# huggingface/tokenizers

Measured on AMD Instinct MI355X. Metric: GB input text/sec (whole node), GPT-2 BPE encode_batch, higher is better.
Workload: dtype u8->u32

## Files before the change

### tokenizers_amd/csrc/capi/handle.cpp

```cpp

struct Workspace {
    std::mutex mu;
    std::function<uint32_t(uint32_t)> pad_exchange;
    uint32_t h_padmax = 0;
    bool busy = false;
    bool device_bound = false;
    hipStream_t bound_stream = nullptr;
    hipStream_t own_stream = nullptr;
    hipStream_t io_in = nullptr, io_out = nullptr;
    hipEvent_t ev_in[2] = {nullptr, nullptr}, ev_out[2] = {nullptr, nullptr};
    DevBuf w_l3_tiles;
    DevBuf w_ms_dmask, w_pprefix, w_pt_word;
    DevBuf w_docmask, w_startmask, w_wprefix, w_bsum, w_tile_w, w_pt_start, w_tok0, w_pt_tokoff, w_tmp_ids, w_tmp_end, w_rows;
    DevBuf w_len1, w_fin, w_fbsum, w_pad_count, w_keep, w_type_ids2, w_seq_ids2;
    DevBuf w_ovf_parts, w_enc_base, w_enc_doc, w_enc_start, w_enc_cnt;
    DevBuf w_enc_idx, w_enc_win;
    DevBuf w_queues, w_qcount, w_cstate;
    DevBuf w_doc_off;
    DevBuf w_chunk_lo;
    DevBuf w_ids, w_doc_pt, w_tok_offsets, w_scalars, w_offsets, w_word_ids;
    DevBuf dw_ids, dw_tok_off, dw_first, dw_bad, dw_dup, dw_len, dw_bsum, dw_pos, dw_out_off, dw_bytes, dw_total;
    DevBuf w_endmask, w_pt_end, w_keepmask, w_kprefix, w_ntext, w_norig, w_ndoc_off, w_slow_docs, w_leadmask, w_lprefix, w_need, w_need_bsum, w_huge, w_list_huge, w_wbase, w_norig_e, w_ids2, w_tok_offsets2, w_offsets2, w_word_ids2, w_candmask, w_matchmask, w_spanmask, w_stopmask, w_hardmask, w_boundmask, w_bprefix, w_seg_off, w_xseg_off,
        w_match_docs, w_match_list;
    DevBuf h_text, h_doc_off, h_seq_off, h_inp_off;
    DevBuf w_tok_b8;
    DevBuf w_trim1;
    const uint8_t* cur_trim1 = nullptr;
    DevBuf w_cache_keys, w_cache_rows;
    DevBuf w_claims, w_claim_rows, w_claim_pos;
    DevBuf w_phases;
    uint64_t cache_epoch = 0;
    DevBuf w_seq_off, w_seq_tok_off, w_word_idx, w_first_tok;
    std::vector<StageRec> pending;
    const uint8_t* last_text = nullptr;
    const int64_t* last_doc_off = nullptr;
    const int64_t* last_seq_off = nullptr;
    int64_t last_n_seqs = -1;
    const int64_t* last_inp_off = nullptr;
    int64_t last_n_inputs = -1;
    DevBuf w_inp_off;
    DevBuf w_mask_dirty;
    int64_t last_n_bytes = 0;
    uint32_t last_flags = 0;
    tkamd_device_result last_result{};
    int64_t last_n_docs = 0;
    int64_t last_n_enc = -1;
    int last_ntok_slot = 1;
    uint32_t last_counters[CNT_COUNT] = {0};
    bool force_general = false;
    bool force_nfc = false;
    bool last_note_nfc = false;
    bool last_note_added = false;
    bool last_used_claims = false;
    ~Workspace() {
        if (own_stream) (void)hipStreamDestroy(own_stream);
        if (io_in) (void)hipStreamDestroy(io_in);
        if (io_out) (void)hipStreamDestroy(io_out);
        for (int i = 0; i < 2; ++i) {
            if (ev_in[i]) (void)hipEventDestroy(ev_in[i]);
            if (ev_out[i]) (void)hipEventDestroy(ev_out[i]);
        }
    }
};

struct tkamd_tokenizer {
    HostModel hm;
    int device = -1;
    DevTables dt{};
    std::mutex mu;
    std::condition_variable cv;
    std::vector<std::unique_ptr<Workspace>> pool;
    Workspace* last_used = nullptr;
    DevBuf t_ucc1, t_ucc2;
    DevBuf t_uc1, t_uc2, t_byte_id, t_merges, t_long_blob, t_long_off, t_long_id, t_long_table;
    DevBuf t_hot;
    DevBuf t_shortw, t_shortw_k3, t_shortw_disp;
    DevBuf t_char_id;
    DevBuf t_at_id[2], t_at_flags[2], t_at_blob[2], t_at_off[2], t_at_first[2];
    DevBuf t_pp_single, t_pp_single_plain;
    DevBuf t_pp_pair, t_pp_pair_plain;
    DevBuf t_pp_prefix, t_pp_suffix, t_pp_prefix_ty, t_pp_suffix_ty, t_bn1, t_bn2, t_bn_map, t_nfc1, t_nfc2, t_nfc_map, t_merge_disp, t_dec_entry, t_dec_blob, t_trie;
    int n_cu = 256;
    int n_direct = 0;
    int n_hot = 0;
    int cp_grid = 0;
    std::atomic<int> claims_pause{0};
    std::atomic<int> added_spec_pause{0};
    std::atomic<int> nfc_spec_pause{0};
    std::atomic<uint32_t> nfc_reruns{0};
    int nfc_spec_len = 32;
    int added_spec_len = 32;
    int claims_pause_len = 32;
    std::atomic<uint32_t> q16_div{4};
    std::atomic<bool> prof{false};
    std::atomic<bool> encode_special{false};
    std::atomic<bool> word_cache{false};
    std::atomic<uint64_t> cache_epoch{1};
    std::vector<tkamd_stage_time> acc;
    std::vector<int> devices;
    std::vector<std::unique_ptr<tkamd_tokenizer>> replicas;
    std::mutex group_mu;
    std::atomic<int> collect{0};
    std::string collect_note;
    std::vector<std::unique_ptr<DevBuf>> g_root;
    std::vector<void*> rccl_comms;
    int64_t shard_min_bytes = 1 << 20;
    std::vector<double> shard_ms;
    std::vector<int64_t> shard_bytes;
};

constexpr size_t PHASE_WGS = 1 << 17;
constexpr size_t MAX_HOST_WORKSPACES = 4;

struct PinnedBlock {
    void* p = nullptr;
    size_t cap = 0;
};
static std::mutex g_pin_mu;
static std::vector<PinnedBlock> g_pin_free;

static PinnedBlock pinned_get(size_t bytes) {
    if (bytes < 64) bytes = 64;
    {
        std::lock_guard<std::mutex> lk(g_pin_mu);
        size_t best = (size_t)-1;
        for (size_t i = 0; i < g_pin_free.size(); ++i)
            if (g_pin_free[i].cap >= bytes && (best == (size_t)-1 || g_pin_free[i].cap < g_pin_free[best].cap)) best = i;
        if (best != (size_t)-1 && g_pin_free[best].cap <= 2 * bytes + (1u << 20)) {
            PinnedBlock b = g_pin_free[best];
            g_pin_free.erase(g_pin_free.begin() + best);
            return b;
        }
    }
    PinnedBlock b;
    size_t want = bytes + bytes / 8;
    HIP_CHECK(hipHostMalloc(&b.p, want, hipHostMallocPortable));
    b.cap = want;
    return b;
}
static void pinned_put(PinnedBlock b) {
    if (!b.p || g_forked) return;
    std::lock_guard<std::mutex> lk(g_pin_mu);
    if (g_pin_free.size() >= 16) { (void)hipHostFree(b.p); return; }
    g_pin_free.push_back(b);
}

struct tkamd_batch {
    int64_t n_docs = 0, n_tokens = 0;
    PinnedBlock ids, tok_offsets, offsets, word_ids, pad_counts, type_ids, seq_ids, enc_docs, enc_parts;
    bool has_offsets = false, has_words = false, has_pads = false, has_types = false, has_enc_docs = false, has_enc_parts = false;
    ~tkamd_batch() { pinned_put(ids); pinned_put(tok_offsets); pinned_put(offsets); pinned_put(word_ids); pinned_put(pad_counts); pinned_put(type_ids); pinned_put(seq_ids); pinned_put(enc_docs); pinned_put(enc_parts); }
};

struct tkamd_text {
    int64_t n_docs = 0, n_bytes = 0;
    PinnedBlock bytes, doc_offsets;
    ~tkamd_text() { pinned_put(bytes); pinned_put(doc_offsets); }
};
```

### tokenizers_amd/csrc/capi/probes.cpp

```cpp

int tkamd_probe_word(const tkamd_tokenizer* t, const uint8_t* bytes, int32_t len, uint32_t* id, uint32_t* flags) {
    if (!t || !bytes || !id || !flags || len < 0) return set_error(TKAMD_ERR_INVALID, "bad argument");
    const HostModel& hm = t->hm;
    *id = 0;
    *flags = 0;
    if (len == 0 || hm.word_table.empty()) return 0;
    if (len <= WORD_MAX_KEY) {
        uint8_t buf[16] = {0};
        memcpy(buf, bytes, (size_t)len);
        uint64_t lo, hi;
        memcpy(&lo, buf, 8);
        memcpy(&hi, buf + 8, 8);
        const uint32_t h1 = word_hash1(lo, hi, (uint32_t)len, hm.word_seed);
        const WordSlot& sa = hm.word_table[word_slot_a(h1, hm.word_mask)];
        const WordSlot& s = (sa.len == (uint32_t)len && sa.lo == lo && sa.hi == hi) ? sa : hm.word_table[word_slot_b(h1, hm.word_mask)];
        if (s.len != (uint32_t)len || s.lo != lo || s.hi != hi) return 0;
        *id = s.id;
        *flags = s.flags;
        return 1;
    }
    if (hm.long_table.empty()) return 0;
    uint32_t h = fnv1a(bytes, (size_t)len) & hm.long_mask;
    for (;;) {
        const uint32_t e = hm.long_table[h];
// ... 92 lines not shown
    t->encode_special = value != 0;
    for (auto& r : t->replicas) r->encode_special = value != 0;
    return TKAMD_OK;
}

int tkamd_word_cache(tkamd_tokenizer* t, int enable, int clear) {
    if (!t) return set_error(TKAMD_ERR_INVALID, "null argument");
    if (clear) ++t->cache_epoch;
    t->word_cache = enable != 0;
    for (auto& r : t->replicas) { if (clear) ++r->cache_epoch; r->word_cache = enable != 0; }
    return TKAMD_OK;
}

int tkamd_profile_enable(tkamd_tokenizer* t, int on) {
    if (!t) return set_error(TKAMD_ERR_INVALID, "null argument");
    t->prof = on != 0;
    for (auto& r : t->replicas) r->prof = on != 0;
    return TKAMD_OK;
}

int tkamd_profile_read(tkamd_tokenizer* t, tkamd_stage_time* stages, int max_stages, int* n_stages, int reset) {
    if (!t || !n_stages) return set_error(TKAMD_ERR_INVALID, "null argument");
    std::lock_guard<std::mutex> lk(t->mu);
    if (t->device >= 0 && !g_forked) {
        (void)hipSetDevice(t->device);
        for (auto& w : t->pool) drain_profile(t, w.get());
        for (auto& r : t->replicas) {
            std::lock_guard<std::mutex> rl(r->mu);
            (void)hipSetDevice(r->device);
            for (auto& w : r->pool) drain_profile(t, w.get());
        }
        if (!t->replicas.empty()) (void)hipSetDevice(t->device);
    }
    int n = (int)std::min<size_t>(t->acc.size(), (size_t)std::max(0, max_stages));
    for (int i = 0; i < n && stages; ++i) stages[i] = t->acc[i];
    *n_stages = n;
    if (reset) t->acc.clear();
    return TKAMD_OK;
}

int tkamd_pinned_alloc(size_t bytes, void** out) {
    if (!out) return set_error(TKAMD_ERR_INVALID, "null argument");
    *out = nullptr;
    return guarded([&]() -> int {
        check_not_forked();
        void* p = nullptr;
        note_hip_used();
        HIP_CHECK(hipHostMalloc(&p, bytes ? bytes : 64, hipHostMallocPortable));
        *out = p;
        return TKAMD_OK;
    });
}
void tkamd_pinned_free(void* p) {
    if (p && !g_forked) (void)hipHostFree(p);
}

int tkamd_debug_phases(tkamd_tokenizer* t, int which, uint64_t* out, int reset) {
    if (!t || !out || which < 0 || which > 1) return set_error(TKAMD_ERR_INVALID, "bad argument");
    return guarded([&]() -> int {
        for (int k = 0; k < 8; ++k) out[k] = 0;
        if (t->device < 0 || g_forked) return TKAMD_OK;
        HIP_CHECK(hipSetDevice(t->device));
        HIP_CHECK(hipDeviceSynchronize());
        std::lock_guard<std::mutex> lk(t->mu);
        std::vector<uint64_t> h(PHASE_WGS * 8);
        for (auto& w : t->pool) {
            if (!w->w_phases.p) continue;
            uint8_t* const p = (uint8_t*)w->w_phases.p + (size_t)which * PHASE_WGS * 64;
            HIP_CHECK(hipMemcpy(h.data(), p, PHASE_WGS * 64, hipMemcpyDeviceToHost));
            for (size_t g = 0; g < PHASE_WGS; ++g)
                for (int k = 0; k < 8; ++k) out[k] += h[g * 8 + k];
            if (reset) HIP_CHECK(hipMemset(p, 0, PHASE_WGS * 64));
        }
        return TKAMD_OK;
    });
}

int tkamd_profile_counters(tkamd_tokenizer* t, uint32_t* out, int n) {
    if (!t || !out) return set_error(TKAMD_ERR_INVALID, "null argument");
    return guarded([&]() -> int {
        std::lock_guard<std::mutex> lk(t->mu);
        Workspace* w = t->last_used;
        for (int i = 0; i < n; ++i) out[i] = 0;
        if (!w) return TKAMD_OK;
        for (int i = 0; i < n && i < CNT_COUNT; ++i) out[i] = w->last_counters[i];
        if (n > 13) out[13] = (uint32_t)pair_merge_occupancy();
        if (n > 14) out[14] = (uint32_t)std::max(0, t->added_spec_pause.load());
        if (n > 15) out[15] = t->q16_div;
        if (n > 16) out[16] = (uint32_t)std::max(0, t->nfc_spec_pause.load());
        if (n > 17) out[17] = t->nfc_reruns.load();
        if (t->device >= 0 && w->w_qcount.p && !g_forked) {
            HIP_CHECK(hipSetDevice(t->device));
            HIP_CHECK(hipDeviceSynchronize());
            std::vector<uint32_t> c(QCNT_WORDS);
            HIP_CHECK(hipMemcpy(c.data(), w->w_qcount.p, (size_t)QCNT_WORDS * 4, hipMemcpyDeviceToHost));
            static const int slot[4] = {CNT_LIST16, CNT_LIST32, CNT_LIST64, CNT_LISTL};
            for (int q = 0; q < 4; ++q) {
                uint32_t sum = 0;
                for (int i = 0; i < NSQ; ++i) sum += c[((size_t)q * NSQ + i) * QCNT_STRIDE];
                if (slot[q] < n) out[slot[q]] = sum;
            }
        }
        return TKAMD_OK;
    });
}

}
#pragma GCC visibility pop
```

### tokenizers_amd/csrc/capi/tables.cpp

```cpp

namespace {

enum { SC_NPRETOK = 0, SC_NTOK = 1, SC_ERR = 2 , SC_NKEPT = 3, SC_PADMAX = 4 , SC_NSEG = 5, SC_NENC = 6, SC_NCHARS = 8, SC_HUGE_USED = 9, SC_NTOK2 = 10, SC_NPIECE = 11,
       SC_COUNTERS = 16 , SC_SLOTS = 32 };

struct Prof {
    tkamd_tokenizer* t;
    Workspace* w;
    hipStream_t st;
    static bool trace() { static const bool on = getenv("TKAMD_TRACE") != nullptr; return on; }
    void begin(const char* name) {
        if (trace()) fprintf(stderr, "[tkamd] %s ...\n", name);
        if (!t->prof) return;
        StageRec r;
        r.name = name;
        HIP_CHECK(hipEventCreate(&r.a));
        HIP_CHECK(hipEventCreate(&r.b));
        HIP_CHECK(hipEventRecord(r.a, st));
        w->pending.push_back(r);
    }
    void end() {
        if (trace()) { HIP_CHECK(hipStreamSynchronize(st)); fprintf(stderr, "[tkamd]   done\n"); }
        if (!t->prof) return;
        HIP_CHECK(hipEventRecord(w->pending.back().b, st));
// ... 90 lines not shown
    d.long_id = t->t_long_id.as<uint32_t>();
    d.long_table = t->t_long_table.as<uint32_t>();
    d.long_mask = hm.long_mask;
    d.trie = t->t_trie.as<MergeSlot>();
    d.trie_mask = hm.trie.mask;
    d.trie_seed = hm.trie.seed;
    d.max_input_chars = hm.max_input_chars;
    d.char_id = nullptr;
    d.cb = 0u;
    if (hm.char_bpe) {
        upload(t->t_char_id, hm.char_id);
        d.char_id = t->t_char_id.as<uint32_t>();
        d.cb = CB_ON | (hm.bpe_prefix.empty() ? 0u : CB_PREFIX) | (hm.bpe_suffix.empty() ? 0u : CB_SUFFIX) | (hm.has_unk ? CB_UNK : 0u) |
               ((hm.unk_configured && !hm.has_unk) ? CB_UNK_MISSING : 0u) | (hm.fuse_unk ? CB_FUSE : 0u) | (hm.byte_fallback ? CB_BYTES : 0u);
    }
}

void verify_direct_words(tkamd_tokenizer* t) {
    HostModel& hm = t->hm;
    if (hm.model != MODEL_BPE || hm.n_words == 0) return;
    std::vector<uint8_t> text;
    std::vector<uint32_t> starts, slot_of;
    for (uint32_t sidx = 0; sidx <= hm.word_mask; ++sidx) {
        const WordSlot& s = hm.word_table[sidx];
        if (s.len == 0) continue;
        uint8_t buf[16];
        memcpy(buf, &s.lo, 8);
        memcpy(buf + 8, &s.hi, 8);
        starts.push_back((uint32_t)text.size());
        slot_of.push_back(sidx);
        text.insert(text.end(), buf, buf + s.len);
    }
    uint32_t P = (uint32_t)starts.size();
    starts.push_back((uint32_t)text.size());
    size_t n = text.size();
    text.resize(n + TKAMD_TEXT_PAD, 0);
    std::vector<uint32_t> items(2 * (size_t)P);
    for (uint32_t i = 0; i < P; ++i) { items[2 * i] = starts[i]; items[2 * i + 1] = starts[i + 1] - starts[i]; }
    DevBuf d_text, d_items, d_n, d_rows, d_tmp;
    upload(d_text, text);
    upload(d_items, items);
    std::vector<uint32_t> nn((size_t)NSQ * QCNT_STRIDE, 0u);
    nn[0] = P;
    upload(d_n, nn);
    d_rows.reserve((size_t)P * 16 + 16);
    d_tmp.reserve(n * 4 + 64);
    HIP_CHECK(hipMemset(d_rows.p, 0, (size_t)P * 16));
    const QView v{(QItem*)d_items.p, d_n.as<uint32_t>(), P, 0u};
    if (hm.char_bpe) {
        DevBuf d_errs, d_hl;
        d_errs.reserve(64);
        d_hl.reserve(64);
        HIP_CHECK(hipMemset(d_errs.p, 0, 64));
        HIP_CHECK(hipMemset(d_hl.p, 0, 64));
        DevTables vt = t->dt;
        vt.err = d_errs.as<int>();
        if (vt.newid_affine) launch_bpe_merge(nullptr, t->n_cu, 5, vt, d_text.as<uint8_t>(), v, d_rows.p, d_tmp.as<uint32_t>(), nullptr);
        else launch_bpe_merge_long_only(nullptr, t->n_cu * 2, vt, d_text.as<uint8_t>(), v, d_rows.p, d_tmp.as<uint32_t>(), nullptr, d_hl.as<uint32_t>(), d_hl.as<uint32_t>() + 4);
        HIP_CHECK(hipGetLastError());
        HIP_CHECK(hipDeviceSynchronize());
    } else
    launch_bpe_merge(nullptr, std::max(1, (int)std::min<uint32_t>(P / 16 + 1, 4096)), 16, t->dt, d_text.as<uint8_t>(), v, d_rows.p, d_tmp.as<uint32_t>(), nullptr);
    HIP_CHECK(hipGetLastError());
    HIP_CHECK(hipDeviceSynchronize());
    std::vector<uint32_t> rows(4 * (size_t)P);
    HIP_CHECK(hipMemcpy(rows.data(), d_rows.p, (size_t)P * 16, hipMemcpyDeviceToHost));
    int nd = 0;
    for (uint32_t i = 0; i < P; ++i) {
        WordSlot& s = hm.word_table[slot_of[i]];
        const uint32_t r0 = rows[4 * (size_t)i];
        const bool one_own = r0 == (s.id | (1u << 28)) ||
                             (r0 == (s.id | (15u << 28)) && rows[4 * (size_t)i + 2] == 1u);
        if (one_own) { s.flags |= WORD_DIRECT; ++nd; }
        else s.flags &= ~WORD_DIRECT;
    }
    t->n_direct = nd;
}

void build_shortw_table(tkamd_tokenizer* t) {
    HostModel& hm = t->hm;
    std::vector<const WordSlot*> ws;
    for (const WordSlot& w : hm.word_table)
        if (w.len) ws.push_back(&w);
    const size_t x10 = 13;
    const uint32_t n_buckets = ws.size() > 65536 ? 4u * (uint32_t)SHORTW_BUCKETS : (uint32_t)SHORTW_BUCKETS;
    uint32_t cap = 16;
    while (cap < ws.size() * x10 / 10) cap <<= 1;
    std::vector<uint32_t> h1(ws.size()), km(ws.size()), where(ws.size());
    for (size_t i = 0; i < ws.size(); ++i) {
        h1[i] = word_hash1(ws[i]->lo, ws[i]->hi, ws[i]->len, hm.word_seed);
        km[i] = shortw_kmix((uint32_t)ws[i]->lo, (uint32_t)(ws[i]->lo >> 32), (uint32_t)ws[i]->hi, (uint32_t)(ws[i]->hi >> 32));
    }
    std::vector<std::vector<uint32_t>> buckets((size_t)n_buckets);
    for (size_t i = 0; i < ws.size(); ++i) buckets[h1[i] & (n_buckets - 1u)].push_back((uint32_t)i);
    std::vector<uint32_t> order((size_t)n_buckets);
    for (uint32_t b = 0; b < n_buckets; ++b) order[b] = b;
    std::stable_sort(order.begin(), order.end(), [&](uint32_t x, uint32_t y) { return buckets[x].size() > buckets[y].size(); });
    std::vector<uint8_t> disp;
    for (;;) {
        std::vector<uint8_t> used((size_t)cap, 0);
        disp.assign((size_t)n_buckets, 0);
        bool ok = true;
        std::vector<uint32_t> slots;
        for (uint32_t b : order) {
            const std::vector<uint32_t>& keys = buckets[b];
            if (keys.empty()) break;
            bool placed = false;
            for (uint32_t d = 0; d < 256u && !placed; ++d) {
                slots.clear();
                bool clash = false;
                for (uint32_t i : keys) {
                    const uint32_t sl = shortw_slot(h1[i], km[i], d, cap - 1);
                    if (used[sl] || std::find(slots.begin(), slots.end(), sl) != slots.end()) { clash = true; break; }
                    slots.push_back(sl);
                }
                if (clash) continue;
                for (size_t k = 0; k < keys.size(); ++k) { used[slots[k]] = 1; where[keys[k]] = slots[k]; }
                disp[b] = (uint8_t)d;
                placed = true;
            }
            if (!placed) { ok = false; break; }
        }
        if (ok) break;
        if (cap >= (1u << 26)) throw Invalid("could not build the short-word hash table");
        cap <<= 1;
    }
    std::vector<HotSlot> tab(cap, HotSlot{0u, 0u, 0u, 0u});
    std::vector<uint32_t> k3(cap, 0u);
    for (size_t i = 0; i < ws.size(); ++i) {
        const WordSlot* w = ws[i];
        if (w->id > SHORTW_ID_MASK) throw Invalid("token id beyond 24 bits");
        tab[where[i]] = HotSlot{(uint32_t)w->lo, (uint32_t)(w->lo >> 32), (uint32_t)w->hi, w->id | (w->len << SHORTW_LEN_SHIFT) | ((w->flags & WORD_DIRECT) ? SHORTW_DIRECT : 0u)};
    }
    for (size_t i = 0; i < ws.size(); ++i) k3[where[i]] = (uint32_t)(ws[i]->hi >> 32);
    upload(t->t_shortw, tab, 64);
    upload(t->t_shortw_k3, k3, 64);
    t->dt.shortw_k3 = t->t_shortw_k3.as<uint32_t>();
    upload(t->t_shortw_disp, disp, 64);
    t->dt.shortw = t->t_shortw.p;
    t->dt.shortw_disp = t->t_shortw_disp.as<uint8_t>();
    t->dt.shortw_mask = cap - 1;
    t->dt.shortw_bmask = n_buckets - 1u;
}

void build_hot_table(tkamd_tokenizer* t) {
    HostModel& hm = t->hm;
    const uint32_t slots = (uint32_t)HOT_SLOTS, n_buckets = slots / 4u;
    std::vector<HotSlot> hot(slots, HotSlot{0u, 0u, 0u, 0u});
    std::vector<uint16_t> disp(n_buckets, 0);
    std::vector<const WordSlot*> cand;
    const bool all_final = hm.model != MODEL_BPE || hm.ignore_merges;
    for (const WordSlot& w : hm.word_table)
        if (w.len && w.len <= (uint32_t)HOT_MAX_KEY && (all_final || (w.flags & WORD_DIRECT))) cand.push_back(&w);
    std::sort(cand.begin(), cand.end(), [](const WordSlot* a, const WordSlot* b) { return a->id < b->id; });
    if (cand.size() > (size_t)slots * 15 / 16) cand.resize((size_t)slots * 15 / 16);
    auto hash_of = [&](const WordSlot* w) { return hot_hash((uint32_t)w->lo, (uint32_t)(w->lo >> 32), (uint32_t)w->hi, w->len, hm.word_seed); };
    std::vector<std::vector<const WordSlot*>> buckets(n_buckets);
    for (const WordSlot* w : cand) buckets[hot_bucket(hash_of(w), slots)].push_back(w);
    std::vector<uint32_t> order(n_buckets);
    for (uint32_t i = 0; i < n_buckets; ++i) order[i] = i;
    std::stable_sort(order.begin(), order.end(), [&](uint32_t a, uint32_t b) { return buckets[a].size() > buckets[b].size(); });
    int n = 0;
    for (uint32_t bi : order) {
        std::vector<const WordSlot*>& bk = buckets[bi];
        while (!bk.empty()) {
            uint32_t d = 0;
            for (; d < slots; ++d) {
                bool ok = true;
                for (size_t i = 0; i < bk.size() && ok; ++i) {
                    const uint32_t s = hot_slot(hash_of(bk[i]), d, slots);
                    ok = hot[s].id_len == 0u;
                    for (size_t j = 0; j < i && ok; ++j) ok = hot_slot(hash_of(bk[j]), d, slots) != s;
                }
                if (ok) break;
            }
            if (d < slots) {
                disp[bi] = (uint16_t)d;
                for (const WordSlot* w : bk) hot[hot_slot(hash_of(w), d, slots)] = HotSlot{(uint32_t)w->lo, (uint32_t)(w->lo >> 32), (uint32_t)w->hi, w->id | (w->len << 24)};
                n += (int)bk.size();
                break;
            }
            bk.pop_back();
        }
    }
    t->n_hot = n;
    std::vector<uint8_t> blob((size_t)hot_table_bytes((int)slots));
    memcpy(blob.data(), hot.data(), (size_t)slots * 16);
    memcpy(blob.data() + (size_t)slots * 16, disp.data(), (size_t)n_buckets * 2);
    upload(t->t_hot, blob);
}
```

### tokenizers_amd/csrc/kernels.hpp

```cpp
#pragma once
#include <hip/hip_runtime_api.h>
#include <cstdint>

#include "nfc_core.hpp"
#include "tables.hpp"

namespace tkamd {

struct DevTables {
    const uint16_t* uc1;
    const uint8_t* uc2;
    const uint32_t* byte_id;
    const MergeSlot* merges;
    const uint16_t* merge_disp;
    uint32_t merge_mask, merge_seed, merge_bmask;
    uint32_t newid_affine, newid_base;
    const uint32_t* char_id;
    uint32_t cb;
    int* err;
    uint32_t* probes;
    void* pub_rows;
    uint32_t* pub_pos;
    uint32_t pub_mask;
    uint32_t word_seed;
    const void* shortw;
    const uint32_t* shortw_k3;
    const uint8_t* shortw_disp;
    uint32_t shortw_mask;
    uint32_t shortw_bmask;
    uint32_t ignore_merges;
    uint32_t long_probe_max_len;
    uint32_t unk_id, has_unk;
    const uint8_t* long_blob;
    const uint32_t* long_off;
    const uint32_t* long_id;
    const uint32_t* long_table;
    uint32_t long_mask;
    const MergeSlot* trie;
    uint32_t trie_mask, trie_seed;
    uint32_t max_input_chars;
};

struct BnTables {
    const uint16_t* bn1;
    const uint8_t* bn2;
    const MergeSlot* map;
    uint32_t map_mask, map_seed;
    uint32_t clean, cjk, strip, lower;
};

struct QItem;
constexpr int NSQ = 768;
constexpr int QCNT_STRIDE = 1;
constexpr int LOOKUP_TILE_BYTES = 16384;
constexpr int QCNT_WORDS = 4 * NSQ * QCNT_STRIDE;
struct QView {
    QItem* q;
    uint32_t* counts;
    uint32_t sq_cap;
    uint32_t row_base;
};
constexpr int WORD_CACHE_BITS = 20;
constexpr uint32_t ROW_INDEX_LIMIT = 1u << 30;
constexpr uint32_t CACHE_CLAIMED = 0x80000000u;
struct __attribute__((aligned(32))) CacheKey {
    uint32_t k[4];
    uint32_t state;
    uint32_t pad[3];
};
struct WordCache {
    CacheKey* keys;
    void* rows;
    unsigned long long* claims;
    uint32_t claim_mask;
    uint32_t* claim_pos;
};

struct ZeroRegions {
    void* p[6];
    unsigned long long n16[6];
    int n;
    const uint32_t* only_if;
    void add(void* ptr, size_t bytes) { if (n < 6 && ptr && bytes) { p[n] = ptr; n16[n] = (bytes + 15) / 16; ++n; } }
};
struct QueuePlan {
    QView v[4];
};

constexpr int META_TILE = 1024;
struct MetaArgs {
    const uint8_t* x_text;
    const uint8_t* text;
    const uint32_t* pt_start;
    const uint32_t* pt_end;
    const unsigned long long* startmask;
    const unsigned long long* endmask;
    const uint32_t* wprefix;
    const uint32_t* tile_w;
    int64_t n_mask_words;
    const int64_t* x_len_dev;
    int64_t x_len_host;
    const int64_t* n_tok;
    const uint32_t* pt_tokoff;
    const uint32_t* tmp_end;
    const uint8_t* tok_b8;
    const uint32_t* tok0;
    const uint32_t* claim_pos;
    const int64_t* n_pretok;
    const uint32_t* doc_pt;
    const uint32_t* chunk_lo;
// ... 276 lines not shown
```

### tokenizers_amd/csrc/kernels/lookup.hip

```cpp

constexpr int LU_NT = 512;
constexpr int LU_WAVES = LU_NT / 64;
constexpr int LU_TILE_WORDS = 256;
constexpr int LU_TILE = LU_TILE_WORDS * 64;
static_assert(LU_TILE == LOOKUP_TILE_BYTES, "the host sizes the sub-queues per tile (capi.cpp queue_sizes)");
constexpr int LU_TEXT_SLACK = 64;
constexpr int HOT = HOT_SLOTS;
constexpr int LU_POS_CAP = 3072;
constexpr int LU_WAVES_PER_SIMD = 6;
constexpr uint32_t CLAIM_ADAPT_MIN = 768u;

struct LookupArgs {
    const uint8_t* text;
    int64_t n_bytes_host;
    const int64_t* len_dev;
    const unsigned long long* startmask;
    const unsigned long long* endmask;
    const uint32_t* wprefix;
    uint32_t* tok0;
    QView v[4];
    int* err;
    const unsigned long long* matchmask;
    const uint4* hot;
    uint32_t word_seed;
    const uint4* shortw;
    const uint32_t* shortw_k3;
    const uint8_t* shortw_disp;
    uint32_t shortw_mask;
    uint32_t shortw_bmask;
    uint32_t any_hit_final;
    uint32_t no_hits;
    uint32_t miss_is_unk;
    uint32_t unk_id, has_unk;
    const CacheKey* cache_keys;
    unsigned long long* claims;
    uint32_t claim_mask;
    uint32_t* counters;
    unsigned long long* phases;
};
enum { LU_PH_STAGE = 0, LU_PH_EXPAND = 1, LU_PH_PASS1 = 2, LU_PH_PASS2 = 3, LU_PH_PASS3 = 4, LU_PH_TOTAL = 7 };

__device__ __forceinline__ uint32_t cache_slot(uint32_t h1) { return (word_hash2(h1) >> 7) & ((1u << WORD_CACHE_BITS) - 1u); }

template <bool HAS_END, bool PROF = false>
__global__ __launch_bounds__(LU_NT, LU_WAVES_PER_SIMD) void k_lookup(LookupArgs a) {
    HIP_DYNAMIC_SHARED(__attribute__((aligned(16))) uint8_t, lu_lds)
    uint4* s_hot = (uint4*)lu_lds;
    uint16_t* s_hdisp = (uint16_t*)(s_hot + HOT);
    uint32_t* s_text32 = (uint32_t*)(s_hdisp + HOT / 4);
    uint16_t* s_pos = (uint16_t*)(s_text32 + (LU_TILE + LU_TEXT_SLACK) / 4 + 4);
    uint16_t* s_miss = s_pos + LU_POS_CAP + 2;
    uint16_t* s_end = s_miss + LU_POS_CAP;
    static_assert(hot_table_bytes(HOT) % 16 == 0, "the text behind the hot table is 16-byte aligned");
    __shared__ uint4 s_kmask[17];
    __shared__ uint32_t s_n, s_pbase, s_last_end, s_nmiss, s_ncand, s_ncandl, s_nretry;
    __shared__ uint32_t s_seen, s_shared, s_claims_on;
    __shared__ uint32_t s_fill[4];
    const int tid = (int)threadIdx.x, lane = tid & 63, wave = tid >> 6;
    unsigned long long ph_t = 0ull, ph_t0 = 0ull, ph_acc[7] = {0ull, 0ull, 0ull, 0ull, 0ull, 0ull, 0ull};
    auto tick = [&](int k) {
        if (PROF && tid == 0) { const unsigned long long now = __builtin_amdgcn_s_memtime(); ph_acc[k] += now - ph_t; ph_t = now; }
    };
    if (PROF && tid == 0) ph_t = ph_t0 = __builtin_amdgcn_s_memtime();
    const uint32_t sq = blockIdx.x;
    if (tid < 4) s_fill[tid] = 0u;
    if (tid == 0) { s_seen = 0u; s_shared = 0u; s_claims_on = a.claims ? 1u : 0u; }
    static_assert(hot_table_bytes(HOT) % 16 == 0, "whole 16-byte words");
    for (int i = tid; i < hot_table_bytes(HOT) / 16; i += LU_NT) s_hot[i] = a.hot[i];
    const uint8_t* const wdisp = a.shortw_disp;
    if (tid < 17) {
        const uint32_t l = (uint32_t)tid;
        auto m = [&](uint32_t lo) -> uint32_t { return l >= lo + 4u ? 0xFFFFFFFFu : (l > lo ? ((1u << (8u * (l - lo))) - 1u) : 0u); };
        s_kmask[tid] = make_uint4(m(0u), m(4u), m(8u), m(12u));
    }
    const int64_t n_bytes = uniform_i64(a.len_dev ? *a.len_dev : a.n_bytes_host);
    const int64_t total_words = (n_bytes + 63) >> 6;
    const int64_t end_words = (n_bytes >> 6) + 1;
    const int64_t n_tiles = (total_words + LU_TILE_WORDS - 1) / LU_TILE_WORDS;
    constexpr bool has_end = HAS_END;
    const bool hits_on = a.no_hits == 0u;
    const int64_t readable = a.n_bytes_host + TEXT_PAD;
    const int half = tid & 1, hword = tid >> 1;
    constexpr int LU_SLACK_CHUNKS = LU_TEXT_SLACK / 16;
    static_assert((LU_TILE + LU_TEXT_SLACK) / 16 == 2 * LU_NT + LU_SLACK_CHUNKS, "two 16-byte text chunks per lane (+ the slack chunks of the first lanes)");
    static_assert(LU_NT == 2 * LU_TILE_WORDS, "two lanes per mask word");
    unsigned long long pf_ms = 0ull, pf_me = 0ull, pf_scan = 0ull;
    uint32_t pf_wp = 0u, pf_first = 0u;
    auto load_text = [&](int64_t tile, Unaligned16& x0, Unaligned16& x1, Unaligned16& xs) {
        x0 = x1 = xs = Unaligned16{0u, 0u, 0u, 0u};
        if (tile >= n_tiles) return;
        const int64_t t0 = (tile * LU_TILE_WORDS) << 6;
        const uint8_t* const tb = uniform_ptr(a.text + t0);
        const uint32_t room = (uint32_t)min(readable - t0, (int64_t)(LU_TILE + LU_TEXT_SLACK + 64));
        const uint32_t g0 = 16u * (uint32_t)tid, g1 = g0 + 16u * (uint32_t)LU_NT, gs = 16u * (uint32_t)(2 * LU_NT + tid);
        if (g0 + 16u <= room) x0 = load_nt16(tb + g0);
        if (g1 + 16u <= room) x1 = load_nt16(tb + g1);
        if (tid < LU_SLACK_CHUNKS && gs + 16u <= room) xs = load_nt16(tb + gs);
    };
    auto prefetch = [&](int64_t tile) {
        pf_ms = pf_me = pf_scan = 0ull;
        pf_wp = pf_first = 0u;
        if (tile >= n_tiles) return;
        const int64_t w0 = tile * LU_TILE_WORDS;
        const int words_left = (int)min(total_words - w0, (int64_t)(LU_TILE_WORDS + 64)), ends_left = (int)min(end_words - w0, (int64_t)(LU_TILE_WORDS + 64));
        const unsigned long long* const sm0 = uniform_ptr(a.startmask + w0);
        const unsigned long long* const em0 = has_end ? uniform_ptr(a.endmask + w0) : sm0;
        const uint32_t* const wp0 = uniform_ptr(a.wprefix + w0);
        if (hword < words_left) { pf_ms = load_nt(sm0 + (uint32_t)hword); pf_wp = load_nt(wp0 + (uint32_t)hword); }
        if (has_end && hword < ends_left) pf_me = load_nt(em0 + (uint32_t)hword);
        pf_first = wp0[0];
        if (wave == 0) {
            const uint32_t ws = (uint32_t)(LU_TILE_WORDS + lane);
            if ((int)ws < (has_end ? ends_left : words_left)) pf_scan = em0[ws];
        }
    };
    prefetch(blockIdx.x);
    for (int64_t tile = blockIdx.x; tile < n_tiles; tile += gridDim.x) {
        const int64_t w0 = tile * LU_TILE_WORDS;
        const int64_t t0 = w0 << 6;
        __syncthreads();
        tick(LU_PH_PASS3);
        if (tid == 0 && s_claims_on && s_seen >= CLAIM_ADAPT_MIN && s_shared * 8u < s_seen) s_claims_on = 0u;
        const unsigned long long ms = pf_ms, me = pf_me;
        uint32_t rbase = 0xFFFFFFFFu;
        {
            const int wl = (int)min(total_words - w0, (int64_t)(LU_TILE_WORDS + 64));
            if (hword < wl) rbase = pf_wp - pf_first;
            if (tid == 0) s_pbase = pf_first;
            if (half && hword < wl && (hword == wl - 1 || hword == LU_TILE_WORDS - 1)) s_n = rbase + (uint32_t)__popcll(ms);
        }
        Unaligned16 tx0, tx1, txs;
        load_text(tile, tx0, tx1, txs);
        auto stage_text = [&]() {
            ((uint4*)s_text32)[tid] = make_uint4(tx0.a, tx0.b, tx0.c, tx0.d);
            ((uint4*)s_text32)[tid + LU_NT] = make_uint4(tx1.a, tx1.b, tx1.c, tx1.d);
            if (tid < LU_SLACK_CHUNKS) ((uint4*)s_text32)[2 * LU_NT + tid] = make_uint4(txs.a, txs.b, txs.c, txs.d);
        };
        if (wave == 0) {
            const unsigned long long* mk = has_end ? a.endmask : a.startmask;
            const int64_t lim = has_end ? end_words : total_words;
            int64_t w = w0 + LU_TILE_WORDS;
            uint32_t found = (uint32_t)n_bytes;
            unsigned long long m = pf_scan;
            while (w < lim) {
                const uint64_t any = __ballot(m != 0ull);
                if (any) {
                    const int l = __ffsll((unsigned long long)any) - 1;
                    const unsigned long long mm = ((unsigned long long)(uint32_t)__shfl((int)(m >> 32), l, 64) << 32) | (uint32_t)__shfl((int)(uint32_t)m, l, 64);
                    found = (uint32_t)(((w + l) << 6) + (__ffsll(mm) - 1));
                    break;
                }
                w += 64;
// ... 340 lines not shown
```

### tokenizers_amd/csrc/tables.hpp

```cpp
#pragma once
#include <cstdint>

#if defined(__HIPCC__)
#include <hip/hip_runtime.h>
#define TK_HD __host__ __device__ __forceinline__
#else
#define TK_HD inline
#endif

namespace tkamd {

enum : uint8_t {
    UC_ONIG_L = 1,
    UC_ONIG_N = 2,
    UC_ONIG_S = 4,
    UC_RX_W = 8,
    UC_RX_S = 16,
    UC_RUST_WS = 32,
    UC_BERT_P = 64,
};

constexpr int UC_STAGE1_LEN = 0x1100;

struct MergeSlot {
    uint32_t a, b, rank, new_id;
};
constexpr uint32_t MERGE_EMPTY = 0xFFFFFFFFu;
constexpr uint32_t RANK_NONE = 0xFFFFFFFFu;

TK_HD uint32_t mix32(uint32_t x) {
    x ^= x >> 16;
    x *= 0x7FEB352Du;
    x ^= x >> 15;
    x *= 0x846CA68Bu;
    x ^= x >> 16;
    return x;
}
TK_HD uint32_t mul24(uint32_t a, uint32_t b) {
#if defined(__HIP_DEVICE_COMPILE__)
    return __umul24(a, b);
#else
    return (uint32_t)(((uint64_t)(a & 0xFFFFFFu) * (uint64_t)(b & 0xFFFFFFu)) & 0xFFFFFFFFull);
#endif
}
TK_HD uint32_t merge_hash1(uint32_t a, uint32_t b, uint32_t seed) {
    const uint32_t k1 = 0x9E3779u ^ (seed & 0xFFFFFEu), k2 = 0x85EBCBu ^ ((seed >> 7) & 0xFFFFFEu);
    const uint32_t x = mul24(a, k1) + mul24(b, k2);
    return x ^ (x >> 15);
}
TK_HD uint32_t merge_hash2(uint32_t a, uint32_t b, uint32_t seed) {
    const uint32_t k3 = 0xC2B2AFu ^ ((seed >> 3) & 0xFFFFFEu), k4 = 0x165667u ^ ((seed >> 11) & 0xFFFFFEu);
    const uint32_t y = mul24(a, k3) + mul24(b, k4) + 0x5BD1E995u;
    return y ^ (y >> 13);
}

constexpr uint32_t PH_MULT = 0x9E3779u;
constexpr int DISP_LDS_MAX = 16384;
TK_HD uint32_t ph_slot(uint32_t h2, uint32_t d, uint32_t mask) { return (h2 + mul24(d, PH_MULT)) & mask; }

struct WordSlot {
    uint64_t lo, hi;
    uint32_t len;
    uint32_t id;
    uint32_t flags;
    uint32_t pad;
};
constexpr uint32_t WORD_DIRECT = 1u;
constexpr int WORD_MAX_KEY = 16;

TK_HD uint32_t hot_hash(uint32_t k0, uint32_t k1, uint32_t k2, uint32_t len, uint32_t seed);
TK_HD uint32_t word_hash1_from_hot(uint32_t hot, uint32_t k3) { return mix32(hot ^ (k3 * 0x165667B1u)); }
TK_HD uint32_t word_hash1(uint64_t lo, uint64_t hi, uint32_t len, uint32_t seed);
TK_HD uint32_t word_hash2(uint32_t h1) { return (h1 * 0x9E3779B1u) ^ (h1 >> 15); }
TK_HD uint32_t word_slot_a(uint32_t h1, uint32_t mask) { return h1 & mask; }
TK_HD uint32_t word_slot_b(uint32_t h1, uint32_t mask) {
    const uint32_t b = (word_hash2(h1) >> 9) & mask;
    return b == (h1 & mask) ? (b ^ 1u) : b;
}

constexpr uint32_t SHORTW_DIRECT = 0x80000000u;
constexpr uint32_t SHORTW_LEN_SHIFT = 24, SHORTW_LEN_MASK = 0x1Fu, SHORTW_ID_MASK = 0xFFFFFFu;
constexpr int SHORTW_BUCKETS = 8192;
TK_HD uint32_t shortw_kmix(uint32_t k0, uint32_t k1, uint32_t k2, uint32_t k3) { return (k0 * 0x85EBCA77u) ^ (k1 * 0xC2B2AE3Du) ^ (k2 * 0x27D4EB2Fu) ^ (k3 * 0x165667B1u); }
TK_HD uint32_t shortw_slot(uint32_t h1, uint32_t kmix, uint32_t d, uint32_t mask) {
    const uint32_t base = ((h1 * 0x9E3779B1u) ^ (h1 >> 15)) ^ kmix, step = ((kmix * 0x9E3779B1u) >> 9) | 1u;
    return (base + d * step) & mask;
}

constexpr int HOT_MAX_KEY = 12;
constexpr int HOT_SLOTS = 1024;
struct HotSlot {
    uint32_t k0, k1, k2, id_len;
};
TK_HD uint32_t hot_bucket(uint32_t h, uint32_t slots) { return h & (slots / 4u - 1u); }
TK_HD uint32_t hot_slot(uint32_t h, uint32_t d, uint32_t slots) { return ((h >> 12) + d) & (slots - 1u); }
constexpr int hot_table_bytes(int slots) { return slots * 16 + slots / 4 * 2; }
TK_HD uint32_t hot_hash(uint32_t k0, uint32_t k1, uint32_t k2, uint32_t len, uint32_t seed) {
    uint32_t h = ((k0 + seed) * 0x9E3779B1u) ^ ((k1 ^ seed) * 0x85EBCA77u) ^ ((k2 + (seed >> 7)) * 0xC2B2AE3Du) ^ (len * 0x27D4EB2Fu);
    h ^= h >> 15;
    h *= 0x2C1B3C6Du;
    return h ^ (h >> 12);
}

TK_HD uint32_t word_hash1(uint64_t lo, uint64_t hi, uint32_t len, uint32_t seed) {
    return word_hash1_from_hot(hot_hash((uint32_t)lo, (uint32_t)(lo >> 32), (uint32_t)hi, len, seed), (uint32_t)(hi >> 32));
}

constexpr uint32_t CHAR_NONE = 0xFFFFFFFFu;
constexpr uint32_t CHAR_TABLE_WORDS = 0x110000u * 4u;
enum : uint32_t {
    CB_ON = 1,
    CB_PREFIX = 2,
    CB_SUFFIX = 4,
    CB_UNK = 8,
    CB_UNK_MISSING = 16,
    CB_FUSE = 32,
    CB_BYTES = 64,
};

TK_HD uint32_t long_key_hash_step(uint32_t h, uint32_t w) {
    h = (h ^ w) * 0x01000193u;
    return h ^ (h >> 15);
}
TK_HD uint32_t long_key_hash_init(uint32_t len) { return 2166136261u ^ (len * 0x9E3779B1u); }

constexpr uint32_t DEC_SPECIAL = 0x80000000u;
constexpr uint32_t DEC_ABSENT = 0x40000000u;
constexpr uint32_t DEC_BYTE = 0x20000000u;
constexpr uint32_t DEC_LEN_MASK = 0x1FFFFFFFu;

enum ModelKind { MODEL_NONE = 0, MODEL_BPE = 1, MODEL_WORDPIECE = 2, MODEL_WORDLEVEL = 3 };
enum PretokKind {
    PT_NONE = 0,
    PT_BYTELEVEL_GPT2 = 1,
    PT_LLAMA3 = 2,
    PT_WHITESPACE = 3,
    PT_WHITESPACE_SPLIT = 4,
    PT_BERT = 5,
    PT_BYTELEVEL_NOREGEX = 6,
    PT_METASPACE = 7,
    PT_SPLIT_CHAIN = 8
};
enum NormKind { NORM_NONE = 0, NORM_BERT = 1, NORM_METASPACE = 2, NORM_NFC = 3 };
enum MsPrepend {
    MS_NEVER = 0,
    MS_ALWAYS = 1,
    MS_FIRST = 2,
    MS_PIECE = 3,
};

struct SplitRule {
    uint8_t contr;
    uint8_t letters;
    uint8_t digit_max;
    uint8_t other_tail;
};
constexpr SplitRule SPLIT_RULE_LLAMA3 = {1, 0, 3, 1};
TK_HD bool split_rule_fast(const SplitRule& r) { return r.letters == 0 && r.other_tail == 1 && r.contr <= 2; }
TK_HD bool split_rule_fast_cs(const SplitRule& r) { return r.letters == 2 && (r.contr == 0 || r.contr == 3); }
enum : uint8_t { UC2_P = 1 , UC2_S = 2 , UC2_M = 4 , UC2_CJK = 8  };
enum : uint8_t { UCC_UPPER = 1 , UCC_LOWER = 2  };

}
```

### tokenizers_amd/tokenizer.py

```python
from __future__ import annotations

import ctypes as C
import json
import os
import re
import threading
from typing import Iterable, Sequence

import numpy as np

from . import _lib
from ._lib import DeviceError, TokenizersAmdError, UnsupportedError


try:
    from . import _marshal
except ImportError:
    _marshal = None


_FORKED = [False]
os.register_at_fork(after_in_child=lambda: _FORKED.__setitem__(0, True))


# ... 843 lines not shown
                if not (isinstance(sq, (list, tuple)) and all(isinstance(x, str) for x in sq)):
                    raise TypeError("is_pretokenized=True: every sequence must be a list of str (TextInputSequence / PreTokenizedInputSequence)")
                words.extend(sq)
                seq_off.append(len(words))
            seqs = words
        elif not all(isinstance(x, str) for x in seqs):
            raise UnsupportedError("a batch holds single sequences (str) and pairs (str, str); lists of words need is_pretokenized=True")
        flags = self._flags(offsets, word_ids, add_special_tokens, False, overflowing)
        inp = np.asarray(inp_off, dtype=np.int64)
        b = C.c_void_p()
        with self._stage_lock:
            buf, doc_off = self._pack_staged(seqs)
            so = np.asarray(seq_off, dtype=np.int64) if seq_off is not None else None
            _lib.check(self._lib.tkamd_encode_batch_mixed(self._h, buf.ctypes.data, doc_off.ctypes.data, len(doc_off) - 1,
                                                          so.ctypes.data if so is not None else None, len(so) - 1 if so is not None else -1,
                                                          inp.ctypes.data, len(inputs), flags, C.byref(b)))
        return self._wrap_batch(b, len(inputs), offsets, word_ids, add_special_tokens, True, kinds)

    def encode_batch(self, input: Iterable[str], is_pretokenized: bool = False, add_special_tokens: bool = True) -> BatchEncoding:
        return self._encode_any(input, "char", True, add_special_tokens, is_pretokenized)

    def encode_batch_fast(self, input: Iterable[str], is_pretokenized: bool = False, add_special_tokens: bool = True) -> BatchEncoding:
        return self._encode_any(input, "none", False, add_special_tokens, is_pretokenized)

    def decode_batch_csr(self, ids: np.ndarray, tok_offsets: np.ndarray, skip_special_tokens: bool = True) -> tuple[np.ndarray, np.ndarray]:
        ids = np.ascontiguousarray(ids, dtype=np.uint32)
        tok_offsets = np.ascontiguousarray(tok_offsets, dtype=np.int64)
        n_docs = len(tok_offsets) - 1
        if n_docs < 0:
            raise ValueError("tok_offsets must hold n_docs + 1 entries")
        b = C.c_void_p()
        flags = _lib.SKIP_SPECIAL if skip_special_tokens else 0
        _lib.check(self._lib.tkamd_decode_batch(self._h, ids.ctypes.data, tok_offsets.ctypes.data, n_docs, flags, C.byref(b)))
        try:
            nb = self._lib.tkamd_text_n_bytes(b)
            raw = np.ctypeslib.as_array(C.cast(self._lib.tkamd_text_bytes(b), C.POINTER(C.c_uint8)), shape=(max(nb, 1),))[:nb].copy()
            off = np.ctypeslib.as_array(C.cast(self._lib.tkamd_text_doc_offsets(b), C.POINTER(C.c_int64)), shape=(n_docs + 1,)).copy()
        finally:
            self._lib.tkamd_text_free(b)
        return raw, off

    def decode_token(self, token_id: int, first_position: bool = False) -> tuple[bytes, int]:
        ln, fl = C.c_int32(0), C.c_int32(0)
        buf = (C.c_uint8 * 4096)()
        _lib.check(self._lib.tkamd_decode_token(self._h, int(token_id), int(first_position), buf, 4096, C.byref(ln), C.byref(fl)))
        return bytes(buf[:min(ln.value, 4096)]), fl.value

    def decode_batch(self, sequences: Sequence[Sequence[int]], skip_special_tokens: bool = True) -> list[str]:
        ids, off = pack_id_sequences(sequences)
        raw, doff = self.decode_batch_csr(ids, off, skip_special_tokens)
        buf = raw.tobytes()
        return [buf[doff[i]:doff[i + 1]].decode("utf-8", "replace") for i in range(len(sequences))]

    def decode(self, ids: Sequence[int], skip_special_tokens: bool = True) -> str:
        return self.decode_batch([ids], skip_special_tokens)[0]

    def encode_batch_device(self, d_text_ptr: int, d_doc_offsets_ptr: int, n_docs: int, n_bytes: int,
                            offsets: str = "none", word_ids: bool = False, stream: int = 0, unsynced: bool = False) -> DeviceBatch:
        flags = {"none": _lib.OFFSETS_NONE, "byte": _lib.OFFSETS_BYTE, "char": _lib.OFFSETS_CHAR}[offsets]
        if word_ids:
            flags |= _lib.WANT_WORD_IDS
        if unsynced:
            flags |= _lib.NO_SPECULATION
        res = _lib.DeviceResult()
        _lib.check(self._lib.tkamd_encode_batch_device(self._h, d_text_ptr, d_doc_offsets_ptr, n_docs, n_bytes, flags,
                                                       stream, C.byref(res)))
        return DeviceBatch(self, res, n_docs, stream, capacity=int(res.ids_capacity))

    def word_cache(self, enable: bool = True, clear: bool = False) -> None:
        _lib.check(self._lib.tkamd_word_cache(self._h, 1 if enable else 0, 1 if clear else 0))
        self._word_cache_on = bool(enable)

    def shard_stats(self) -> list[tuple[int, int, float]]:
        n = max(len(self.devices), 1)
        nb, ms, k = (C.c_int64 * n)(), (C.c_double * n)(), C.c_int(0)
        _lib.check(self._lib.tkamd_shard_stats(self._h, nb, ms, n, C.byref(k)))
        return [(self.devices[i], nb[i], ms[i]) for i in range(min(k.value, n))]

    def profile(self, on: bool) -> None:
        _lib.check(self._lib.tkamd_profile_enable(self._h, 1 if on else 0))
        self._profile_on = bool(on)

    def queue_sizes(self) -> dict[str, int]:
        arr = (C.c_uint32 * 18)()
        _lib.check(self._lib.tkamd_profile_counters(self._h, arr, 18))
        out = {"merge16": arr[0], "merge32": arr[3], "merge64": arr[1], "merge_long": arr[2], "pretok_slow_docs": arr[4], "merge_huge": arr[7]}
        if arr[5]:
            out["claim_candidates"], out["claim_shared"] = arr[5], arr[6]
        out["added_spec_pause"] = arr[14]
        out["nfc_spec_pause"], out["nfc_reruns"] = arr[16], arr[17]
        out["merge_pair_wg_per_cu"] = arr[13]
        out["q16_div"] = arr[15]
        if arr[12]:
            out["merge_probes"] = arr[12]
        return out

    def debug_phases(self, reset: bool = True) -> dict[str, list[int]]:
        out = {}
        for which, name in ((0, "lookup"), (1, "compact")):
            arr = (C.c_uint64 * 8)()
            _lib.check(self._lib.tkamd_debug_phases(self._h, which, arr, 1 if reset else 0))
            out[name] = list(arr)
        return out

    def profile_read(self, reset: bool = True) -> dict[str, tuple[float, int]]:
        arr = (_lib.StageTime * _lib.MAX_STAGES)()
        n = C.c_int(0)
        _lib.check(self._lib.tkamd_profile_read(self._h, arr, _lib.MAX_STAGES, C.byref(n), 1 if reset else 0))
        return {arr[i].name.decode(): (arr[i].ms_total, arr[i].launches) for i in range(n.value)}
```

Measured before the change: 271.8.

## Rebuild short-word perfect hash with load-factor sizing and 16-bit displacements

Reworks construction of the short-word displacement hash table. Slot capacity now targets a load factor near 0.96 instead of about 0.77, and the bucket count scales with the vocabulary instead of being fixed at 8192 or 32768. Displacements widen from 8 to 16 bits so that denser placements can succeed. The intent is a smaller table that stays in cache better during lookup, at the cost of a larger displacement array, longer host build time, and an extra 2-byte load per probe. New counters expose the table sizes and the largest displacement.

```diff
diff --git a/tokenizers_amd/csrc/capi/handle.cpp b/tokenizers_amd/csrc/capi/handle.cpp
--- a/tokenizers_amd/csrc/capi/handle.cpp
+++ b/tokenizers_amd/csrc/capi/handle.cpp
@@ -83,6 +83,7 @@
     int n_cu = 256;
     int n_direct = 0;
     int n_hot = 0;
+    uint32_t shortw_max_disp = 0;
     int cp_grid = 0;
     std::atomic<int> claims_pause{0};
     std::atomic<int> added_spec_pause{0};
diff --git a/tokenizers_amd/csrc/capi/probes.cpp b/tokenizers_amd/csrc/capi/probes.cpp
--- a/tokenizers_amd/csrc/capi/probes.cpp
+++ b/tokenizers_amd/csrc/capi/probes.cpp
@@ -198,6 +198,10 @@
         std::lock_guard<std::mutex> lk(t->mu);
         Workspace* w = t->last_used;
         for (int i = 0; i < n; ++i) out[i] = 0;
+        if (n > 18) out[18] = t->dt.shortw ? t->dt.shortw_mask + 1u : 0u;
+        if (n > 19) out[19] = t->dt.shortw ? t->dt.shortw_bmask + 1u : 0u;
+        if (n > 20) out[20] = t->shortw_max_disp;
+        if (n > 21) out[21] = (uint32_t)t->hm.merge_table.size();
         if (!w) return TKAMD_OK;
         for (int i = 0; i < n && i < CNT_COUNT; ++i) out[i] = w->last_counters[i];
         if (n > 13) out[13] = (uint32_t)pair_merge_occupancy();
diff --git a/tokenizers_amd/csrc/capi/tables.cpp b/tokenizers_amd/csrc/capi/tables.cpp
--- a/tokenizers_amd/csrc/capi/tables.cpp
+++ b/tokenizers_amd/csrc/capi/tables.cpp
@@ -196,31 +196,32 @@
     std::vector<const WordSlot*> ws;
     for (const WordSlot& w : hm.word_table)
         if (w.len) ws.push_back(&w);
-    const size_t x10 = 13;
-    const uint32_t n_buckets = ws.size() > 65536 ? 4u * (uint32_t)SHORTW_BUCKETS : (uint32_t)SHORTW_BUCKETS;
+    const size_t n = ws.size();
     uint32_t cap = 16;
-    while (cap < ws.size() * x10 / 10) cap <<= 1;
-    std::vector<uint32_t> h1(ws.size()), km(ws.size()), where(ws.size());
-    for (size_t i = 0; i < ws.size(); ++i) {
+    while ((uint64_t)cap * 24u < (uint64_t)n * 25u) cap <<= 1;
+    uint32_t nb_first = 16;
+    while ((size_t)nb_first * 8u < n) nb_first <<= 1;
+    std::vector<uint32_t> h1(n), km(n), where(n);
+    for (size_t i = 0; i < n; ++i) {
         h1[i] = word_hash1(ws[i]->lo, ws[i]->hi, ws[i]->len, hm.word_seed);
         km[i] = shortw_kmix((uint32_t)ws[i]->lo, (uint32_t)(ws[i]->lo >> 32), (uint32_t)ws[i]->hi, (uint32_t)(ws[i]->hi >> 32));
     }
-    std::vector<std::vector<uint32_t>> buckets((size_t)n_buckets);
-    for (size_t i = 0; i < ws.size(); ++i) buckets[h1[i] & (n_buckets - 1u)].push_back((uint32_t)i);
-    std::vector<uint32_t> order((size_t)n_buckets);
-    for (uint32_t b = 0; b < n_buckets; ++b) order[b] = b;
-    std::stable_sort(order.begin(), order.end(), [&](uint32_t x, uint32_t y) { return buckets[x].size() > buckets[y].size(); });
-    std::vector<uint8_t> disp;
-    for (;;) {
+    std::vector<uint16_t> disp;
+    std::vector<std::vector<uint32_t>> buckets;
+    std::vector<uint32_t> order, slots;
+    auto place = [&](uint32_t n_buckets) -> bool {
+        buckets.assign((size_t)n_buckets, std::vector<uint32_t>());
+        for (size_t i = 0; i < n; ++i) buckets[h1[i] & (n_buckets - 1u)].push_back((uint32_t)i);
+        order.resize((size_t)n_buckets);
+        for (uint32_t b = 0; b < n_buckets; ++b) order[b] = b;
+        std::stable_sort(order.begin(), order.end(), [&](uint32_t x, uint32_t y) { return buckets[x].size() > buckets[y].size(); });
         std::vector<uint8_t> used((size_t)cap, 0);
         disp.assign((size_t)n_buckets, 0);
-        bool ok = true;
-        std::vector<uint32_t> slots;
         for (uint32_t b : order) {
             const std::vector<uint32_t>& keys = buckets[b];
             if (keys.empty()) break;
             bool placed = false;
-            for (uint32_t d = 0; d < 256u && !placed; ++d) {
+            for (uint32_t d = 0; d < 65536u && !placed; ++d) {
                 slots.clear();
                 bool clash = false;
                 for (uint32_t i : keys) {
@@ -230,15 +231,22 @@
                 }
                 if (clash) continue;
                 for (size_t k = 0; k < keys.size(); ++k) { used[slots[k]] = 1; where[keys[k]] = slots[k]; }
-                disp[b] = (uint8_t)d;
+                disp[b] = (uint16_t)d;
                 placed = true;
             }
-            if (!placed) { ok = false; break; }
+            if (!placed) return false;
         }
-        if (ok) break;
+        return true;
+    };
+    uint32_t n_buckets = nb_first;
+    for (;;) {
+        if (place(n_buckets)) break;
+        if ((size_t)n_buckets * 2u * 2u <= n) { n_buckets <<= 1; continue; }
         if (cap >= (1u << 26)) throw Invalid("could not build the short-word hash table");
         cap <<= 1;
-    }
+        n_buckets = nb_first;
+    }
+    t->shortw_max_disp = disp.empty() ? 0u : (uint32_t)*std::max_element(disp.begin(), disp.end());
     std::vector<HotSlot> tab(cap, HotSlot{0u, 0u, 0u, 0u});
     std::vector<uint32_t> k3(cap, 0u);
     for (size_t i = 0; i < ws.size(); ++i) {
@@ -252,7 +260,7 @@
     t->dt.shortw_k3 = t->t_shortw_k3.as<uint32_t>();
     upload(t->t_shortw_disp, disp, 64);
     t->dt.shortw = t->t_shortw.p;
-    t->dt.shortw_disp = t->t_shortw_disp.as<uint8_t>();
+    t->dt.shortw_disp = t->t_shortw_disp.as<uint16_t>();
     t->dt.shortw_mask = cap - 1;
     t->dt.shortw_bmask = n_buckets - 1u;
 }
diff --git a/tokenizers_amd/csrc/kernels.hpp b/tokenizers_amd/csrc/kernels.hpp
--- a/tokenizers_amd/csrc/kernels.hpp
+++ b/tokenizers_amd/csrc/kernels.hpp
@@ -25,7 +25,7 @@
     uint32_t word_seed;
     const void* shortw;
     const uint32_t* shortw_k3;
-    const uint8_t* shortw_disp;
+    const uint16_t* shortw_disp;
     uint32_t shortw_mask;
     uint32_t shortw_bmask;
     uint32_t ignore_merges;
diff --git a/tokenizers_amd/csrc/kernels/lookup.hip b/tokenizers_amd/csrc/kernels/lookup.hip
--- a/tokenizers_amd/csrc/kernels/lookup.hip
+++ b/tokenizers_amd/csrc/kernels/lookup.hip
@@ -25,7 +25,7 @@
     uint32_t word_seed;
     const uint4* shortw;
     const uint32_t* shortw_k3;
-    const uint8_t* shortw_disp;
+    const uint16_t* shortw_disp;
     uint32_t shortw_mask;
     uint32_t shortw_bmask;
     uint32_t any_hit_final;
@@ -67,7 +67,7 @@
     if (tid == 0) { s_seen = 0u; s_shared = 0u; s_claims_on = a.claims ? 1u : 0u; }
     static_assert(hot_table_bytes(HOT) % 16 == 0, "whole 16-byte words");
     for (int i = tid; i < hot_table_bytes(HOT) / 16; i += LU_NT) s_hot[i] = a.hot[i];
-    const uint8_t* const wdisp = a.shortw_disp;
+    const uint16_t* const wdisp = a.shortw_disp;
     if (tid < 17) {
         const uint32_t l = (uint32_t)tid;
         auto m = [&](uint32_t lo) -> uint32_t { return l >= lo + 4u ? 0xFFFFFFFFu : (l > lo ? ((1u << (8u * (l - lo))) - 1u) : 0u); };
diff --git a/tokenizers_amd/csrc/tables.hpp b/tokenizers_amd/csrc/tables.hpp
--- a/tokenizers_amd/csrc/tables.hpp
+++ b/tokenizers_amd/csrc/tables.hpp
@@ -80,7 +80,6 @@
 
 constexpr uint32_t SHORTW_DIRECT = 0x80000000u;
 constexpr uint32_t SHORTW_LEN_SHIFT = 24, SHORTW_LEN_MASK = 0x1Fu, SHORTW_ID_MASK = 0xFFFFFFu;
-constexpr int SHORTW_BUCKETS = 8192;
 TK_HD uint32_t shortw_kmix(uint32_t k0, uint32_t k1, uint32_t k2, uint32_t k3) { return (k0 * 0x85EBCA77u) ^ (k1 * 0xC2B2AE3Du) ^ (k2 * 0x27D4EB2Fu) ^ (k3 * 0x165667B1u); }
 TK_HD uint32_t shortw_slot(uint32_t h1, uint32_t kmix, uint32_t d, uint32_t mask) {
     const uint32_t base = ((h1 * 0x9E3779B1u) ^ (h1 >> 15)) ^ kmix, step = ((kmix * 0x9E3779B1u) >> 9) | 1u;
diff --git a/tokenizers_amd/tokenizer.py b/tokenizers_amd/tokenizer.py
--- a/tokenizers_amd/tokenizer.py
+++ b/tokenizers_amd/tokenizer.py
@@ -949,8 +949,8 @@
         self._profile_on = bool(on)
 
     def queue_sizes(self) -> dict[str, int]:
-        arr = (C.c_uint32 * 18)()
-        _lib.check(self._lib.tkamd_profile_counters(self._h, arr, 18))
+        arr = (C.c_uint32 * 22)()
+        _lib.check(self._lib.tkamd_profile_counters(self._h, arr, 22))
         out = {"merge16": arr[0], "merge32": arr[3], "merge64": arr[1], "merge_long": arr[2], "pretok_slow_docs": arr[4], "merge_huge": arr[7]}
         if arr[5]:
             out["claim_candidates"], out["claim_shared"] = arr[5], arr[6]
@@ -958,6 +958,7 @@
         out["nfc_spec_pause"], out["nfc_reruns"] = arr[16], arr[17]
         out["merge_pair_wg_per_cu"] = arr[13]
         out["q16_div"] = arr[15]
+        out["shortw_slots"], out["shortw_buckets"], out["shortw_max_disp"], out["merge_slots"] = arr[18], arr[19], arr[20], arr[21]
         if arr[12]:
             out["merge_probes"] = arr[12]
         return out
```

Result: faster. 274.7 (median of 6 runs) (+1.0%).
